# at-cg/PHI

Hardware: AMD Instinct MI355X
Metric: read Gbases/s scored (49-hap MHC graph stand-in synMHC-49); reads resident in HBM, parsing and H2D excluded (higher is better)
Workload: dtype u64

## Files before the change

phi_amd/csrc/contexts.hip:

```cpp
#include <hip/hip_runtime.h>
#include "phi_dev.h"
#include "phi_kernels.h"
#include "phi_wave.h"

static inline unsigned grid_for(int64_t n, int tpb)
{
    int64_t nb = (n + tpb - 1) / tpb;
    if (nb > 256 * 32) nb = 256 * 32;
    if (nb < 1) nb = 1;
    return (unsigned)nb;
}

#define GRID_STRIDE(i, n) \
    for (int64_t i = (int64_t)blockIdx.x * blockDim.x + threadIdx.x; i < (n); i += (int64_t)gridDim.x * blockDim.x)

__device__ __forceinline__ int32_t walk_of(const int64_t *__restrict__ walk_off, int32_t n_walks, int64_t e)
{
    int32_t lo = 0, hi = n_walks;
    while (hi - lo > 1) {
        const int32_t mid = (lo + hi) >> 1;
        if (walk_off[mid] <= e) lo = mid; else hi = mid;
    }
    return lo;
}

__global__ void __launch_bounds__(256) phi_vlen_kernel(const int64_t *__restrict__ seq_off, int64_t n_vtx, int32_t *__restrict__ vlen)
{
    GRID_STRIDE(v, n_vtx) vlen[v] = (int32_t)(seq_off[v + 1] - seq_off[v]);
}
void phi_launch_vlen(hipStream_t st, const int64_t *seq_off, int64_t n_vtx, int32_t *vlen)
{
    if (n_vtx > 0) hipLaunchKernelGGL(phi_vlen_kernel, dim3(grid_for(n_vtx, 256)), dim3(256), 0, st, seq_off, n_vtx, vlen);
}

template <bool BY_CLASS>
__global__ void __launch_bounds__(256) phi_walk_sum_kernel(const int32_t *__restrict__ key, const int32_t *__restrict__ val_of,
                                                           const int32_t *__restrict__ cls_rec_off, const int64_t *__restrict__ walk_off,
                                                           int32_t n_walks, int64_t n_entries, unsigned long long *__restrict__ out)
{
    const int64_t n_waves = (int64_t)gridDim.x * (blockDim.x / 64);
    const int64_t gw = (int64_t)blockIdx.x * (blockDim.x / 64) + (threadIdx.x >> 6);
    const int lane = threadIdx.x & 63;
    const int64_t per = ((n_entries + n_waves - 1) / n_waves + 63) & ~(int64_t)63;
    const int64_t lo = gw * per, hi = lo + per < n_entries ? lo + per : n_entries;
    if (lo >= hi) return;
    int32_t h = walk_of(walk_off, n_walks, lo);
    int64_t h_end = walk_off[h + 1];
    long long acc = 0;
    for (int64_t e0 = lo; e0 < hi; e0 += 64) {
        const int64_t e = e0 + lane;
        long long v = 0;
        if (e < hi) {
            const int32_t x = key[e];
            v = BY_CLASS ? (cls_rec_off[x + 1] - cls_rec_off[x]) : val_of[x];
        }
        if (e0 + 64 <= h_end) acc += v;
        else {
            int64_t row_lo = e0;
            for (;;) {
                const long long mine = (e >= row_lo && e < h_end) ? v : 0;
                acc += mine;
                if (h_end >= e0 + 64 || h_end >= hi) break;
                acc = phi_wave_sum(acc);
                if (lane == 0 && acc) atomicAdd(&out[h], (unsigned long long)acc);
                acc = 0;
                row_lo = h_end;
                h++;
                h_end = walk_off[h + 1];
            }
        }
    }
    acc = phi_wave_sum(acc);
    if (lane == 0 && acc) atomicAdd(&out[h], (unsigned long long)acc);
}
static inline unsigned walk_sum_grid(int64_t n_entries)
{
    int64_t nb = (n_entries + 256 * 64 - 1) / (256 * 64);
    if (nb > 1024) nb = 1024;
    return (unsigned)(nb < 1 ? 1 : nb);
}
void phi_launch_walk_bases(hipStream_t st, const int32_t *walk_vtx, const int32_t *vlen, const int64_t *walk_off, int32_t n_walks,
                           int64_t n_entries, unsigned long long *out)
{
    if (n_entries > 0)
        hipLaunchKernelGGL(phi_walk_sum_kernel<false>, dim3(walk_sum_grid(n_entries)), dim3(256), 0, st, walk_vtx, vlen, nullptr,
                           walk_off, n_walks, n_entries, out);
}
void phi_launch_walk_rec_counts(hipStream_t st, const int32_t *ent_cls, const int32_t *cls_rec_off, const int64_t *walk_off,
                                int32_t n_walks, int64_t n_entries, unsigned long long *out)
{
    if (n_entries > 0)
        hipLaunchKernelGGL(phi_walk_sum_kernel<true>, dim3(walk_sum_grid(n_entries)), dim3(256), 0, st, ent_cls, nullptr, cls_rec_off,
                           walk_off, n_walks, n_entries, out);
}

struct EntCtx { int32_t left; int32_t n; int32_t tail; };

__device__ __forceinline__ EntCtx entry_context(const PhiClassArgs &A, int64_t e, int64_t w_lo, int64_t w_hi)
{
    EntCtx c;
    c.left = 256;
    if (e > w_lo) {
        const int32_t pv = A.walk_vtx[e - 1];
        const int64_t pe = A.seq_off[pv + 1];
        c.left = pe > A.seq_off[pv] ? (int32_t)A.seq[pe - 1] : 257;
    }
    c.n = 0; c.tail = 0;
    while (c.tail < A.tail_need && e + c.n + 1 < w_hi) { c.n++; c.tail += A.vlen[A.walk_vtx[e + c.n]]; }
    return c;
}

__device__ __forceinline__ uint64_t context_key(const PhiClassArgs &A, int64_t e, const EntCtx &c)
{
    uint64_t h = A.seed ^ ((uint64_t)(uint32_t)c.left * 0x9E3779B97F4A7C15ull);
    h = phi_fmix64(h ^ (uint64_t)(uint32_t)c.n);
    for (int32_t j = 0; j <= c.n; j++) h = phi_fmix64(h ^ (uint64_t)(uint32_t)A.walk_vtx[e + j]) + 0x632BE59BD9B4E019ull;
    return h == PHI_EMPTY_KEY ? 0 : h;
}

__global__ void __launch_bounds__(256) phi_class_insert_kernel(PhiClassArgs A)
{
    GRID_STRIDE(e, A.n_entries) {
        const int32_t h = walk_of(A.walk_off, A.n_walks, e);
        const EntCtx c = entry_context(A, e, A.walk_off[h], A.walk_off[h + 1]);
        const uint64_t key = context_key(A, e, c);
        uint64_t s = key & A.t_mask;
        int probes = 0;
        for (;;) {
            unsigned long long prev = __builtin_nontemporal_load((const unsigned long long *)&A.t_keys[s]);
            if (prev == PHI_EMPTY_KEY) prev = atomicCAS((unsigned long long *)&A.t_keys[s], PHI_EMPTY_KEY, key);
            if (prev == PHI_EMPTY_KEY || prev == key) break;
            s = (s + 1) & A.t_mask;
            if (++probes > PHI_MAX_PROBE) { atomicOr(A.err, PHI_KERR_TABLE_FULL); break; }
        }
        if (__builtin_nontemporal_load(&A.t_rep[s]) > (uint32_t)e) atomicMin(&A.t_rep[s], (uint32_t)e);
        A.ent_slot[e] = (uint32_t)s;
    }
}

__global__ void __launch_bounds__(256) phi_class_verify_kernel(PhiClassArgs A, uint8_t *__restrict__ is_rep)
{
    GRID_STRIDE(e, A.n_entries) {
        const uint32_t s = A.ent_slot[e];
        const int64_t r = (int64_t)A.t_rep[s];
        is_rep[e] = r == e;
        if (r != e) {
            const int32_t h = walk_of(A.walk_off, A.n_walks, e), hr = walk_of(A.walk_off, A.n_walks, r);
            const int64_t w_hi = A.walk_off[h + 1], r_lo = A.walk_off[hr], r_hi = A.walk_off[hr + 1];
            const EntCtx c = entry_context(A, e, A.walk_off[h], w_hi);
            int32_t rleft = 256;
            if (r > r_lo) {
                const int32_t pv = A.walk_vtx[r - 1];
                const int64_t pe = A.seq_off[pv + 1];
                rleft = pe > A.seq_off[pv] ? (int32_t)A.seq[pe - 1] : 257;
            }
            bool same = rleft == c.left && r + c.n < r_hi;
            if (same && c.tail < A.tail_need && r + c.n + 1 != r_hi) same = false;
            for (int32_t j = 0; same && j <= c.n; j++) same = A.walk_vtx[r + j] == A.walk_vtx[e + j];
            if (!same) { atomicOr(A.err, PHI_KERR_FP_COLLISION); continue; }
        }
        atomicAdd(&A.t_mult[s], 1u);
    }
}

__global__ void __launch_bounds__(256) phi_class_ids_kernel(const phi_ent_t *__restrict__ cls_rep, int64_t n_cls,
                                                            const uint32_t *__restrict__ ent_slot, const uint32_t *__restrict__ t_mult,
                                                            uint32_t *__restrict__ t_cid, int32_t *__restrict__ cls_mult)
{
    GRID_STRIDE(c, n_cls) {
        const uint32_t s = ent_slot[cls_rep[c]];
        t_cid[s] = (uint32_t)c;
        cls_mult[c] = (int32_t)t_mult[s];
    }
}
__global__ void __launch_bounds__(256) phi_entry_class_kernel(const uint32_t *ent_slot, int64_t n_entries,
                                                              const uint32_t *__restrict__ t_cid, int32_t *ent_cls)
{
    GRID_STRIDE(e, n_entries) ent_cls[e] = (int32_t)t_cid[ent_slot[e]];
}

__global__ void __launch_bounds__(256) phi_class_len_kernel(PhiClassArgs A, const phi_ent_t *__restrict__ cls_rep, int64_t n_cls,
                                                            int32_t *__restrict__ cls_len, uint8_t *__restrict__ cls_left)
{
    GRID_STRIDE(c, n_cls) {
        const int64_t r = cls_rep[c];
        const int32_t h = walk_of(A.walk_off, A.n_walks, r);
        const EntCtx x = entry_context(A, r, A.walk_off[h], A.walk_off[h + 1]);
        const int32_t left = x.left != 256;
        cls_left[c] = (uint8_t)left;
        cls_len[c] = left + A.vlen[A.walk_vtx[r]] + (x.tail < A.tail_need ? x.tail : A.tail_need);
    }
}

void phi_launch_class_insert(hipStream_t st, const PhiClassArgs &A)
{
    if (A.n_entries > 0) hipLaunchKernelGGL(phi_class_insert_kernel, dim3(grid_for(A.n_entries, 256)), dim3(256), 0, st, A);
}
void phi_launch_class_verify(hipStream_t st, const PhiClassArgs &A, uint8_t *is_rep)
{
    if (A.n_entries > 0) hipLaunchKernelGGL(phi_class_verify_kernel, dim3(grid_for(A.n_entries, 256)), dim3(256), 0, st, A, is_rep);
}
void phi_launch_class_ids(hipStream_t st, const phi_ent_t *cls_rep, int64_t n_cls, const uint32_t *ent_slot, int64_t n_entries,
                          const uint32_t *t_mult, uint32_t *t_cid, int32_t *cls_mult, int32_t *ent_cls)
{
    if (n_cls > 0)
        hipLaunchKernelGGL(phi_class_ids_kernel, dim3(grid_for(n_cls, 256)), dim3(256), 0, st, cls_rep, n_cls, ent_slot, t_mult, t_cid, cls_mult);
    if (n_entries > 0)
        hipLaunchKernelGGL(phi_entry_class_kernel, dim3(grid_for(n_entries, 256)), dim3(256), 0, st, ent_slot, n_entries, t_cid, ent_cls);
}
void phi_launch_class_len(hipStream_t st, const PhiClassArgs &A, const phi_ent_t *cls_rep, int64_t n_cls, int32_t *cls_len, uint8_t *cls_left)
{
    if (n_cls > 0) hipLaunchKernelGGL(phi_class_len_kernel, dim3(grid_for(n_cls, 256)), dim3(256), 0, st, A, cls_rep, n_cls, cls_len, cls_left);
}

__global__ void __launch_bounds__(256) phi_pack_classes_kernel(const uint8_t *__restrict__ seq, const int64_t *__restrict__ seq_off,
                                                               const int32_t *__restrict__ walk_vtx, const int32_t *__restrict__ vlen,
                                                               const phi_ent_t *__restrict__ cls_rep, const uint8_t *__restrict__ cls_left,
                                                               const int64_t *__restrict__ cls_base, int64_t n_cls,
                                                               uint64_t *__restrict__ words, int64_t n_words, uint32_t *__restrict__ badbits,
                                                               uint8_t *__restrict__ ascii, unsigned long long *__restrict__ n_bad)
{
    const int64_t wi = (int64_t)blockIdx.x * blockDim.x + threadIdx.x;
    if (wi >= n_words + 4) return;
    if (wi >= n_words) {
        if (wi < n_words + 2) words[wi] = 0;
        if (badbits) badbits[wi] = 0;
        return;
    }
    const int64_t total = cls_base[n_cls];
    const int64_t b0 = wi * 32;
    uint64_t word = 0;
    uint32_t bad = 0;
    if (b0 < total) {
        int64_t c = phi_locate_in(cls_base, n_cls, b0);
        int64_t c_end = cls_base[c + 1];
        int64_t ent = -1, ent_o = 0, ent_end = 0;
        const uint8_t *src = nullptr;
        bool fresh = true;
        for (int j = 0; j < 32; j++) {
            const int64_t b = b0 + j;
            uint32_t ch = 'A';
            if (b < total) {
                while (b >= c_end) { c++; c_end = cls_base[c + 1]; fresh = true; }
                const int64_t o = b - cls_base[c];
                const int left = cls_left[c];
                if (left && o == 0) {
                    const int32_t pv = walk_vtx[cls_rep[c] - 1];
                    ch = seq[seq_off[pv + 1] - 1];
                } else {
                    if (fresh) {
                        ent = cls_rep[c]; ent_o = left;
                        const int32_t v = walk_vtx[ent];
                        ent_end = ent_o + vlen[v];
                        src = seq + seq_off[v] - ent_o;
                        fresh = false;
                    }
                    while (o >= ent_end) {
                        ent++; ent_o = ent_end;
                        const int32_t v = walk_vtx[ent];
                        ent_end = ent_o + vlen[v];
                        src = seq + seq_off[v] - ent_o;
                    }
                    ch = src[o];
                }
                bad |= (uint32_t)(!phi_is_acgt(ch)) << j;
                if (ascii) ascii[b] = (uint8_t)ch;
            }
            word = (word << 2) | phi_code(ch);
        }
    }
    words[wi] = word;
    if (badbits) badbits[wi] = bad;
    if (bad) atomicAdd(n_bad, (unsigned long long)__popc(bad));
}

void phi_launch_pack_classes(hipStream_t st, const uint8_t *seq, const int64_t *seq_off, const int32_t *walk_vtx, const int32_t *vlen,
                             const phi_ent_t *cls_rep, const uint8_t *cls_left, const int64_t *cls_base, int64_t n_cls, uint64_t *words,
                             int64_t n_words, uint32_t *badbits, uint8_t *ascii, unsigned long long *n_bad)
{
    if (n_words <= 0) return;
    const int64_t nb = (n_words + 4 + 255) / 256;
    hipLaunchKernelGGL(phi_pack_classes_kernel, dim3((unsigned)nb), dim3(256), 0, st, seq, seq_off, walk_vtx, vlen, cls_rep, cls_left,
                       cls_base, n_cls, words, n_words, badbits, ascii, n_bad);
// ... 313 lines not shown
```

phi_amd/csrc/phi_kernels.h:

```cpp
#pragma once
#include <stdint.h>
#include <hip/hip_runtime.h>
#include "phi_dp_flags.h"

#ifndef PHI_TPB
#define PHI_TPB 256

#endif
#define PHI_WCH 512
#define PHI_MAX_W 256
#define PHI_MAX_K 64
#define PHI_MAX_K_PACKED 32
#define PHI_MAX_PROBE 4096
#define PHI_RT_OVERFLOWED 1u
static inline int phi_nov_shift(int w)
{
    const int want = (3 * 2 * PHI_WCH) / (2 * (w + 1));
    int sh = 4;
    while ((1 << sh) < want && sh < 9) sh++;
    return sh;
}
#define PHI_STRIPES 256

typedef uint32_t phi_ent_t;
// ... 15 lines not shown
#define PHI_KERR_HASH_COLLISION 128u

struct PhiSketchArgs {
    const uint64_t *words;
    const unsigned long long *starts;
    int64_t n_bases;
    int32_t k, w;
    const unsigned long long *badbits;
    const uint8_t *ascii;
    int32_t allslow;
    int32_t *block_cnt;
    const int64_t *block_off;
    uint64_t *out_hash;
    int64_t *out_pos;
    unsigned long long *n_logged;
    unsigned long long *n_emitted;
    const uint64_t *u_rt; uint64_t u_bmask;
    uint8_t *hit;
    uint32_t *err;
    uint64_t *nov_log; uint16_t *nov_cnt; int64_t log_base; int32_t nov_shift;
    uint64_t *ov_list; unsigned long long *ov_count; int64_t ov_cap;
    const int64_t *read_off; int64_t n_reads;
    uint32_t reads_per_base_q32;
    int32_t uniform_len;
    double inv_len;
    uint32_t inv_len_q32;
    int32_t wave_stride;
    int32_t q_clean;
    int32_t win_reads;
    unsigned long long *ov_zero;
    unsigned long long *ipc_mb; unsigned long long ipc_scored, ipc_need;
    uint64_t *q_hit_words; int64_t q_n_hit_words; uint64_t *q_stripes; int64_t q_n_stripe_words;
    const uint64_t *k_rt; uint64_t k_bmask;
};
#define PHI_NOV_KMERS 0x8000u

void phi_launch_pack_ascii(hipStream_t st, const uint8_t *bases, int64_t n, uint64_t *words, int64_t n_words,
                           uint32_t *badbits, unsigned long long *n_bad);
void phi_launch_mark_starts(hipStream_t st, const int64_t *seq_off, int64_t n_seq, unsigned long long *starts);

void phi_launch_sketch_bytes(hipStream_t st, int mode, const PhiSketchArgs &A, const unsigned long long *batch_bad);
void phi_launch_reset_reads(hipStream_t st, uint64_t *hit_words, int64_t n_hit_words, uint64_t *stripes, int64_t n_stripe_words);
int64_t phi_sketch_num_blocks(int64_t n_bases);
int phi_sketch_win_reads(int k, int w, int64_t uniform_len, int64_t n_reads, int64_t n_bases);
int64_t phi_sketch_read_chunks(int k, int w, int64_t uniform_len, int64_t n_reads, int64_t n_bases);
void phi_launch_sketch(hipStream_t st, int mode, const PhiSketchArgs &A, hipEvent_t t0 = nullptr, hipEvent_t t1 = nullptr);

void phi_launch_table_build(hipStream_t st, const uint64_t *rec_hash, int64_t n_rec, uint64_t *u_keys,
                            uint32_t *u_rep, uint64_t u_mask, uint32_t *rec_slot, uint32_t *err);
void phi_launch_rep_flags(hipStream_t st, const uint32_t *rec_slot, int64_t n_rec, const uint32_t *u_rep,
                          uint8_t *flags);
void phi_launch_table_compact(hipStream_t st, const int32_t *rep_list, int64_t n_unique, const uint64_t *rec_hash, int64_t n_rec,
                              uint64_t *keys, uint32_t *uid, uint64_t mask, uint32_t *rec_slot, uint32_t *err);
void phi_launch_share_hist(hipStream_t st, const uint64_t *keys, int64_t cap, const int32_t *n_walks_of, unsigned long long *hist);
void phi_launch_slot_uid(hipStream_t st, const int32_t *rep_list, int64_t n_unique, const uint32_t *rec_slot,
                         uint32_t *u_uid);
void phi_launch_read_table(hipStream_t st, const uint64_t *keys, const uint32_t *uid, int64_t cap, uint64_t *rt,
                           int64_t n_buckets, uint32_t *err);
void phi_launch_fill_u64(hipStream_t st, uint64_t *p, int64_t n, uint64_t v);
void phi_launch_fill_u32(hipStream_t st, uint32_t *p, int64_t n, uint32_t v);
void phi_launch_iota_i64(hipStream_t st, int64_t *p, int64_t n, int64_t step);
void phi_launch_spectrum_insert(hipStream_t st, const uint64_t *hashes, int64_t n, uint64_t *sp_keys,
                                uint64_t sp_mask, unsigned long long *sp_count, const uint64_t *u_keys, uint64_t u_mask,
                                const uint32_t *u_uid, uint8_t *hit, uint32_t *err);
void phi_launch_spectrum_flush(hipStream_t st, const uint64_t *nov_log, const uint16_t *nov_cnt, int64_t c_lo, int64_t c_hi, int32_t shift,
                               uint64_t *sp_keys, uint64_t sp_mask, unsigned long long *sp_count, int32_t k, const uint64_t *u_keys,
                               uint64_t u_mask, uint32_t *err);
void phi_launch_kmer_keys(hipStream_t st, const int32_t *rec_cls, const int32_t *rec_rel, const uint64_t *rec_hash, const uint32_t *rec_slot,
                          int64_t n_rec, const int64_t *cls_base, const uint8_t *cls_left, const uint64_t *words, const uint32_t *badbits,
                          int32_t k, uint64_t *kkeys, unsigned long long *ctr);
void phi_launch_rt_overflowed(hipStream_t st, const uint64_t *rt, int64_t n_buckets, unsigned long long *n_out);
void phi_launch_count_flags(hipStream_t st, const uint8_t *flags, int64_t n, unsigned long long *n_out);
void phi_launch_spectrum_export(hipStream_t st, const uint64_t *sp_keys, int64_t cap, uint64_t *out,
                                unsigned long long *n_out);

struct PhiClassArgs {
    const int32_t *walk_vtx; const int64_t *walk_off; int32_t n_walks; int64_t n_entries;
    const int32_t *vlen; const uint8_t *seq; const int64_t *seq_off;
    int32_t tail_need;
    uint64_t seed;
    uint64_t *t_keys; uint32_t *t_rep; uint32_t *t_mult; uint64_t t_mask;
    uint32_t *ent_slot;
    uint32_t *err;
};
struct PhiExpandArgs {
    const int32_t *ent_cls; int64_t e_lo, e_hi;
    const int32_t *cls_rec_off; const phi_ent_t *cls_rep;
    const uint8_t *sel; const int32_t *sel_cnt;
    int32_t *block_cnt; const int64_t *block_off;
    const uint64_t *rec_hash; const int32_t *rec_rel; const int64_t *ent_base; uint64_t *out_hash; int64_t *out_pos;
    const uint32_t *rec_slot; const uint32_t *u_uid; const phi_ent_t *rec_e0; const phi_ent_t *rec_e1; uint32_t *out_tri;
};
void phi_launch_vlen(hipStream_t st, const int64_t *seq_off, int64_t n_vtx, int32_t *vlen);
void phi_launch_walk_bases(hipStream_t st, const int32_t *walk_vtx, const int32_t *vlen, const int64_t *walk_off, int32_t n_walks,
                           int64_t n_entries, unsigned long long *out);
void phi_launch_walk_rec_counts(hipStream_t st, const int32_t *ent_cls, const int32_t *cls_rec_off, const int64_t *walk_off,
                                int32_t n_walks, int64_t n_entries, unsigned long long *out);
void phi_launch_class_insert(hipStream_t st, const PhiClassArgs &A);
void phi_launch_class_verify(hipStream_t st, const PhiClassArgs &A, uint8_t *is_rep);
void phi_launch_class_ids(hipStream_t st, const phi_ent_t *cls_rep, int64_t n_cls, const uint32_t *ent_slot, int64_t n_entries,
                          const uint32_t *t_mult, uint32_t *t_cid, int32_t *cls_mult, int32_t *ent_cls);
void phi_launch_class_len(hipStream_t st, const PhiClassArgs &A, const phi_ent_t *cls_rep, int64_t n_cls, int32_t *cls_len, uint8_t *cls_left);
void phi_launch_pack_classes(hipStream_t st, const uint8_t *seq, const int64_t *seq_off, const int32_t *walk_vtx, const int32_t *vlen,
                             const phi_ent_t *cls_rep, const uint8_t *cls_left, const int64_t *cls_base, int64_t n_cls, uint64_t *words,
                             int64_t n_words, uint32_t *badbits, uint8_t *ascii, unsigned long long *n_bad);
void phi_launch_class_rec(hipStream_t st, const int64_t *raw_pos, int64_t n_raw, const int64_t *cls_base, int64_t n_cls,
                          const phi_ent_t *cls_rep, const uint8_t *cls_left, const int32_t *walk_vtx, const int32_t *vlen, int32_t k,
                          uint8_t *keep, int32_t *r_cls, int32_t *r_rel, phi_ent_t *r_e0, phi_ent_t *r_e1);
void phi_launch_class_rec_gather(hipStream_t st, const int32_t *idx, int64_t n, const uint64_t *raw_hash, const int32_t *r_cls,
                                 const int32_t *r_rel, const phi_ent_t *r_e0, const phi_ent_t *r_e1, uint64_t *o_hash, int32_t *o_cls,
                                 int32_t *o_rel, phi_ent_t *o_e0, phi_ent_t *o_e1);
void phi_launch_class_rec_off(hipStream_t st, const int32_t *rec_cls, int64_t n_rec, int64_t n_cls, int32_t *off);
int64_t phi_expand_num_blocks(int64_t n_entries);
void phi_launch_expand_count(hipStream_t st, const PhiExpandArgs &A);
void phi_launch_expand_write(hipStream_t st, const PhiExpandArgs &A, int kind);
void phi_launch_class_sel_count(hipStream_t st, const uint8_t *sel, const int32_t *cls_rec_off, int64_t n_cls, int32_t *sel_cnt);
void phi_launch_class_sel_tri(hipStream_t st, const uint8_t *sel, const int32_t *cls_rec_off, int64_t n_cls, const int32_t *sel_off, const phi_ent_t *cls_rep,
                              const uint32_t *rec_slot, const uint32_t *u_uid, const phi_ent_t *rec_e0, const phi_ent_t *rec_e1, int32_t *sel_tri);
void phi_launch_expand_tri(hipStream_t st, const int32_t *ent_cls, int64_t e_lo, int64_t e_hi, const int32_t *sel_off, const int32_t *sel_tri,
                           const int64_t *block_off, uint32_t *out_tri, phi_ent_t *a_e1, uint8_t *a_span, const int64_t *walk_off, int32_t n_walks,
                           unsigned long long *walk_cnt, unsigned long long *prep, int64_t n_anchors);
void phi_launch_mark_list(hipStream_t st, const int32_t *list, const int32_t *through, int64_t n, uint8_t *sel);
void phi_launch_share_count_cls(hipStream_t st, const int32_t *ent_cls, int64_t e_lo, int64_t e_hi, const int32_t *cls_rec_off,
                                const uint32_t *rec_slot, int32_t walk, int32_t *last_walk, int32_t *n_walks_of);
void phi_launch_entry_len_range(hipStream_t st, const int32_t *walk_vtx, const int32_t *vlen, int64_t e_lo, int64_t n, int32_t *lens);

#define PHI_KERR_FP_COLLISION 8u
void phi_launch_walk_edges(hipStream_t st, const int32_t *walk_vtx, const int64_t *walk_off, int32_t n_walks, int64_t n_entries, int32_t n_vtx,
                           const int64_t *adj_off, const int32_t *adj, const int64_t *seq_off, const int32_t *topo_rank,
                           uint8_t *e_out, int32_t *cnt_edge, unsigned long long *st_mask, int32_t nw64, int32_t *err);
void phi_launch_csr_count(hipStream_t st, const uint32_t *triples, int64_t n, int64_t n_ids, int32_t *cnt, uint32_t *err);
void phi_launch_csr_scatter(hipStream_t st, const uint32_t *triples, int64_t n, int64_t n_ids, const int32_t *off, int32_t *cur,
                            int32_t *idx);
void phi_launch_csr_sort(hipStream_t st, const int32_t *off, int64_t n_ids, int32_t *idx);
void phi_launch_match_flags(hipStream_t st, const uint32_t *rec_slot, int64_t n_rec, const uint32_t *u_uid,
                            const uint8_t *hit, uint8_t *flags);

struct PhiFilterArgs {
    const uint32_t *rec_slot; const phi_ent_t *rec_e0; const phi_ent_t *rec_e1;
    const int32_t *walk_vtx;
    const int32_t *rec_cls; const int32_t *cls_mult;
    const int32_t *m_rec;
    uint64_t *g_keys; int32_t *g_rep; uint32_t *g_cnt; uint64_t g_mask; uint64_t seed;
    int32_t *m_group;
    const uint32_t *u_uid;
    uint32_t *slot_maxcnt;
    uint8_t *slot_multi;
    float limit;
    unsigned long long *counters;
    uint32_t *err;
};
void phi_launch_group_insert(hipStream_t st, const PhiFilterArgs &A, int64_t n_matched);
void phi_launch_group_count(hipStream_t st, const PhiFilterArgs &A, int64_t n_matched);
void phi_launch_group_max(hipStream_t st, const PhiFilterArgs &A, int64_t n_matched);
void phi_launch_slot_count(hipStream_t st, const PhiFilterArgs &A, int64_t u_cap);
void phi_launch_kept_flags(hipStream_t st, const PhiFilterArgs &A, int64_t n_matched, uint8_t *kept, uint8_t *dp);
void phi_launch_gather_i32(hipStream_t st, const int32_t *src, const uint32_t *idx, int64_t n, int32_t *out);
void phi_launch_gather_u64(hipStream_t st, const uint64_t *src, const int32_t *idx, int64_t n, uint64_t *out);
void phi_launch_entry_csr(hipStream_t st, const phi_ent_t *a_e1, int64_t n_a, int64_t n_entries, int64_t *g_off);

#define PHI_DP_CHUNK 128
#define PHI_DP_RING 2048
#define PHI_SCOUT_MAX_WALKS 65535
#define PHI_DP_MAX_WALKS 1022

struct PhiDpArgs {
    int32_t n_vtx, n_walks;
    const int32_t *st_rec;
    const unsigned long long *st_mask;
    const int32_t *in_packed;
    const int64_t *walk_off;
    const uint64_t *word;
    const int64_t *g_off; const uint8_t *g_span; const uint8_t *a_weight;
    int32_t cost;
    int32_t *dmax;
    int32_t *bstart;
    int32_t *tops;
    int32_t *ent_src, *ent_h;
};
void phi_launch_dp(hipStream_t st, const PhiDpArgs &A);
int phi_dp_num_waves(int n_walks);
void phi_launch_dp_words(hipStream_t st, const uint8_t *e_out, const int64_t *g_off, const uint8_t *g_span,
// ... 131 lines not shown
```

phi_amd/csrc/set_graph.hip:

```cpp
#include <string.h>
#include <algorithm>
#include <future>
#include <memory>
#include "phi_ctx.h"
#include "phi_dev.h"
#include "dp_steps.h"

static int build_read_table(phi_ctx *c)
{
    uint64_t nb = pow2_at_least(std::max<uint64_t>(64, (16 * (uint64_t)c->n_unique + 2) / 3));
    if (const char *e = getenv("PHI_READ_TABLE_BUCKETS")) nb = pow2_at_least(std::max<long long>(atoll(e), 1));
    uint32_t err0 = 0;
    HIPCHK(hipMemcpyAsync(&err0, scalar(c, S_ERR), 4, hipMemcpyDeviceToHost, c->stream));
    HIPCHK(hipStreamSynchronize(c->stream));
    for (int attempt = 0;; attempt++) {
        PHICHK(phi_dev_ensure(c, c->d_rt, nb * 32));
        phi_launch_read_table(c->stream, c->d_u_keys.as<uint64_t>(), c->d_u_uid.as<uint32_t>(), (int64_t)c->u_cap,
                              c->d_rt.as<uint64_t>(), (int64_t)nb, (uint32_t *)scalar(c, S_ERR));
        uint32_t err = 0;
        HIPCHK(hipMemcpyAsync(&err, scalar(c, S_ERR), 4, hipMemcpyDeviceToHost, c->stream));
        HIPCHK(hipStreamSynchronize(c->stream));
        if ((err0 & PHI_KERR_TABLE_FULL) || !(err & PHI_KERR_TABLE_FULL)) break;
        if (attempt >= 40) return phi_fail(c, PHI_ERR_OVERFLOW, "read table overflow at %llu buckets (internal error)", (unsigned long long)nb);
        err &= ~PHI_KERR_TABLE_FULL;
        HIPCHK(phi_copy_sync(c, scalar(c, S_ERR), &err, 4, hipMemcpyHostToDevice));
        nb *= 2;
    }
    c->rt_buckets = nb; c->rt_mask = nb - 1;
    return PHI_OK;
}

static int build_kmer_table(phi_ctx *c)
{
    c->kt_buckets = 0; c->kt_mask = 0;
    if (c->k > 31 || c->n_rec <= 0 || c->n_unique <= 0) return PHI_OK;
    PhiStageTimer tg("set_graph");
    DevBuf kkeys, ctr;
    PhiDevGuard guard{{&kkeys, &ctr}};
    PHICHK(phi_dev_ensure(c, kkeys, c->u_cap * 8));
    PHICHK(phi_dev_ensure(c, ctr, 5 * 8));
    phi_launch_fill_u64(c->stream, kkeys.as<uint64_t>(), (int64_t)c->u_cap, PHI_EMPTY_KEY);
    HIPCHK(hipMemsetAsync(ctr.p, 0, 5 * 8, c->stream));
    phi_launch_kmer_keys(c->stream, c->d_rec_cls.as<int32_t>(), c->d_rec_rel.as<int32_t>(), c->d_rec_hash.as<uint64_t>(), c->d_rec_slot.as<uint32_t>(),
                         c->n_rec, c->d_cls_base.as<int64_t>(), c->d_cls_left.as<uint8_t>(), c->d_wwords.as<uint64_t>(), c->d_wbad.as<uint32_t>(),
                         c->k, kkeys.as<uint64_t>(), ctr.as<unsigned long long>());
    uint64_t n[5] = {0, 0, 0, 0, 0};
    HIPCHK(phi_copy_sync(c, n, ctr.p, 3 * 8, hipMemcpyDeviceToHost));
    if (n[1]) return phi_fail(c, PHI_ERR_DEVICE, "k-mer table: %llu class records whose k-mer in class space does not hash to the record's hash (internal error)", (unsigned long long)n[1]);
    if (n[2]) {
        if (tg.on) fprintf(stderr, "[phi timing] set_graph: %llu walk minimisers share a hash with another k-mer: no k-mer table for this graph\n", (unsigned long long)n[2]);
        return PHI_OK;
    }
    uint64_t nb = c->rt_buckets;
    uint32_t err0 = 0;
    HIPCHK(phi_copy_sync(c, &err0, scalar(c, S_ERR), 4, hipMemcpyDeviceToHost));
    if (err0 & PHI_KERR_TABLE_FULL) return PHI_OK;
    for (int attempt = 0;; attempt++) {
        PHICHK(phi_dev_ensure(c, c->d_kt, nb * 32));
        phi_launch_read_table(c->stream, kkeys.as<uint64_t>(), c->d_u_uid.as<uint32_t>(), (int64_t)c->u_cap, c->d_kt.as<uint64_t>(), (int64_t)nb,
                              (uint32_t *)scalar(c, S_ERR));
        uint32_t err = 0;
        HIPCHK(phi_copy_sync(c, &err, scalar(c, S_ERR), 4, hipMemcpyDeviceToHost));
        if (!(err & PHI_KERR_TABLE_FULL)) break;
        if (attempt >= 40) return phi_fail(c, PHI_ERR_OVERFLOW, "k-mer table overflow at %llu buckets (internal error)", (unsigned long long)nb);
        err &= ~PHI_KERR_TABLE_FULL;
        HIPCHK(phi_copy_sync(c, scalar(c, S_ERR), &err, 4, hipMemcpyHostToDevice));
        nb *= 2;
    }
    c->kt_buckets = nb; c->kt_mask = nb - 1;
    int n_cu = 0;
    HIPCHK(hipDeviceGetAttribute(&n_cu, hipDeviceAttributeMultiprocessorCount, c->device));
    c->kt_max_chunks = (int64_t)n_cu * 4 * 7;
    if (tg.on) {
        phi_launch_rt_overflowed(c->stream, c->d_rt.as<uint64_t>(), (int64_t)c->rt_buckets, ctr.as<unsigned long long>() + 3);
        phi_launch_rt_overflowed(c->stream, c->d_kt.as<uint64_t>(), (int64_t)nb, ctr.as<unsigned long long>() + 4);
        HIPCHK(phi_copy_sync(c, n + 3, ctr.as<uint64_t>() + 3, 2 * 8, hipMemcpyDeviceToHost));
        fprintf(stderr, "[phi timing] set_graph: k-mer table of %llu buckets (%.1f MB) beside the read table's %llu; %llu class records with a base outside ACGT skipped; "
                        "OVERFLOWED buckets: read table %.2e, k-mer table %.2e\n", (unsigned long long)nb, (double)nb * 32 / 1e6, (unsigned long long)c->rt_buckets,
                (unsigned long long)n[0], (double)n[3] / (double)c->rt_buckets, (double)n[4] / (double)nb);
        tg.lap("[gpu thread]   k-mer table");
    }
    return PHI_OK;
}

static int build_classes(phi_ctx *c, int32_t n_vtx, int32_t n_walks, int64_t n_entries)
{
    PhiStageTimer tg("set_graph");
    hipEvent_t ev0 = nullptr, ev1 = nullptr;
    HIPCHK(hipEventCreate(&ev0));
    HIPCHK(hipEventCreate(&ev1));
    struct EvGuard { hipEvent_t a, b; ~EvGuard() { (void)hipEventDestroy(a); (void)hipEventDestroy(b); } } evg{ev0, ev1};
    HIPCHK(hipEventRecord(ev0, c->stream));
    PHICHK(phi_dev_ensure(c, c->d_vlen, (size_t)n_vtx * 4));
    phi_launch_vlen(c->stream, c->d_seq_off.as<int64_t>(), n_vtx, c->d_vlen.as<int32_t>());
    PHICHK(phi_dev_ensure(c, c->d_list, (size_t)(n_walks + 1) * 8));
    HIPCHK(hipMemsetAsync(c->d_list.p, 0, (size_t)(n_walks + 1) * 8, c->stream));
    phi_launch_walk_bases(c->stream, c->d_walk_vtx.as<int32_t>(), c->d_vlen.as<int32_t>(), c->d_walk_off.as<int64_t>(), n_walks, n_entries,
                          c->d_list.as<unsigned long long>());
    c->h_walk_base.assign(n_walks + 1, 0);
    HIPCHK(hipMemcpyAsync(c->h_walk_base.data() + 1, c->d_list.p, (size_t)n_walks * 8, hipMemcpyDeviceToHost, c->stream));

    tg.lap("[gpu thread]     events, vlen, walk bases");
    PHICHK(phi_dev_ensure(c, c->d_ent_cls, (size_t)n_entries * 4));
    PHICHK(phi_dev_ensure(c, c->d_flags, (size_t)n_entries));
    DevBuf t_keys, t_rep, t_mult;
    PhiDevGuard guard{{&t_keys, &t_rep, &t_mult}};
    PhiClassArgs A{};
    A.walk_vtx = c->d_walk_vtx.as<int32_t>(); A.walk_off = c->d_walk_off.as<int64_t>(); A.n_walks = n_walks; A.n_entries = n_entries;
    A.vlen = c->d_vlen.as<int32_t>(); A.seq = c->d_seq.as<uint8_t>(); A.seq_off = c->d_seq_off.as<int64_t>();
    A.tail_need = c->w + c->k - 2;
    A.ent_slot = c->d_ent_cls.as<uint32_t>();
    A.err = (uint32_t *)scalar(c, S_ERR);
    const uint64_t cap_max = pow2_at_least(std::max<uint64_t>(1024, 2 * (uint64_t)n_entries));
    uint64_t cap = std::min(cap_max, pow2_at_least(std::max<uint64_t>(1024, 4 * (uint64_t)n_vtx)));
    tg.lap("[gpu thread]     entry buffers");
    for (int attempt = 0;; attempt++) {
        PHICHK(phi_dev_ensure(c, t_keys, cap * 8));
        PHICHK(phi_dev_ensure(c, t_rep, cap * 4));
        PHICHK(phi_dev_ensure(c, t_mult, cap * 4));
        A.t_keys = t_keys.as<uint64_t>(); A.t_rep = t_rep.as<uint32_t>(); A.t_mult = t_mult.as<uint32_t>(); A.t_mask = cap - 1;
        A.seed = 0x13198A2E03707344ull + 0x9E3779B97F4A7C15ull * (uint64_t)attempt;
        phi_launch_fill_u64(c->stream, A.t_keys, (int64_t)cap, PHI_EMPTY_KEY);
        phi_launch_fill_u32(c->stream, A.t_rep, (int64_t)cap, 0xFFFFFFFFu);
        HIPCHK(hipMemsetAsync(A.t_mult, 0, cap * 4, c->stream));
        phi_launch_class_insert(c->stream, A);
        uint32_t err = 0;
        HIPCHK(hipMemcpyAsync(&err, scalar(c, S_ERR), 4, hipMemcpyDeviceToHost, c->stream));
        HIPCHK(hipStreamSynchronize(c->stream));
        if (err & PHI_KERR_TABLE_FULL) {
            if (cap == cap_max) return phi_fail(c, PHI_ERR_OVERFLOW, "walk-context table overflow (internal error)");
            cap = std::min(cap_max, cap * 8);
            err &= ~PHI_KERR_TABLE_FULL;
            HIPCHK(phi_copy_sync(c, scalar(c, S_ERR), &err, 4, hipMemcpyHostToDevice));
            attempt--;
            continue;
        }
        phi_launch_class_verify(c->stream, A, c->d_flags.as<uint8_t>());
        HIPCHK(hipMemcpyAsync(&err, scalar(c, S_ERR), 4, hipMemcpyDeviceToHost, c->stream));
        HIPCHK(hipStreamSynchronize(c->stream));
        if (!(err & PHI_KERR_FP_COLLISION)) break;
        if (attempt >= 7) return phi_fail(c, PHI_ERR_DEVICE, "walk-context fingerprints collide under 8 seeds (internal error)");
        err &= ~PHI_KERR_FP_COLLISION;
        HIPCHK(phi_copy_sync(c, scalar(c, S_ERR), &err, 4, hipMemcpyHostToDevice));
    }
    tg.lap("[gpu thread]     table insert + verify");
    for (int32_t h = 0; h < n_walks; h++) c->h_walk_base[h + 1] += c->h_walk_base[h];
    c->walk_bases = c->h_walk_base[n_walks];
    PHICHK(phi_compact(c, c->d_flags.as<uint8_t>(), n_entries, c->d_cls_rep, &c->n_cls));
    const int64_t nc = c->n_cls;
    tg.lap("[gpu thread]     compact representatives");
    PHICHK(phi_dev_ensure(c, c->d_cls_mult, (size_t)nc * 4));
    PHICHK(phi_dev_ensure(c, c->d_cls_left, (size_t)nc));
    PHICHK(phi_dev_ensure(c, c->d_cls_base, (size_t)(nc + 1) * 8));
    PHICHK(phi_dev_ensure(c, c->d_cls_rec_off, (size_t)(nc + 1) * 4));
    phi_launch_class_ids(c->stream, c->d_cls_rep.as<phi_ent_t>(), nc, A.ent_slot, n_entries, A.t_mult, A.t_rep, c->d_cls_mult.as<int32_t>(),
                         c->d_ent_cls.as<int32_t>());
    PHICHK(phi_dev_ensure(c, c->d_list3, (size_t)nc * 4));
    phi_launch_class_len(c->stream, A, c->d_cls_rep.as<phi_ent_t>(), nc, c->d_list3.as<int32_t>(), c->d_cls_left.as<uint8_t>());
    PHICHK(phi_scan(c, c->d_list3.as<int32_t>(), nc, c->d_cls_base.as<int64_t>()));
    int64_t run = 0;
    HIPCHK(hipMemcpyAsync(&run, c->d_cls_base.as<int64_t>() + nc, 8, hipMemcpyDeviceToHost, c->stream));
    HIPCHK(hipStreamSynchronize(c->stream));
    c->cls_bases = run;
    if (tg.on) fprintf(stderr, "[phi timing] set_graph: %lld entries in %lld classes, %lld bases of class space for %lld bases of walks\\n",
                       (long long)n_entries, (long long)nc, (long long)run, (long long)c->walk_bases);
    tg.lap("[gpu thread]   classes");

    const int64_t n_words = (run + 31) / 32;
    PHICHK(phi_dev_ensure(c, c->d_wwords, (size_t)(n_words + 2) * 8));
    PHICHK(phi_dev_ensure(c, c->d_wbad, (size_t)(n_words + 6) * 4));
    auto pack = [&](uint8_t *ascii) {
        phi_launch_pack_classes(c->stream, c->d_seq.as<uint8_t>(), c->d_seq_off.as<int64_t>(), c->d_walk_vtx.as<int32_t>(), c->d_vlen.as<int32_t>(),
                                c->d_cls_rep.as<phi_ent_t>(), c->d_cls_left.as<uint8_t>(), c->d_cls_base.as<int64_t>(), nc,
                                c->d_wwords.as<uint64_t>(), n_words, c->d_wbad.as<uint32_t>(), ascii, (unsigned long long *)scalar(c, S_NBAD));
    };
    pack(nullptr);
    const uint8_t *cls_ascii = nullptr;
    {
        uint64_t n_bad = 0;
        HIPCHK(hipMemcpyAsync(&n_bad, scalar(c, S_NBAD), 8, hipMemcpyDeviceToHost, c->stream));
        HIPCHK(hipStreamSynchronize(c->stream));
        if (n_bad || c->k > PHI_MAX_K_PACKED) {
            PHICHK(phi_dev_ensure(c, c->d_wascii, (size_t)run + 64));
            HIPCHK(hipMemsetAsync(scalar(c, S_NBAD), 0, 8, c->stream));
            pack(c->d_wascii.as<uint8_t>());
            cls_ascii = c->d_wascii.as<uint8_t>();
        }
    }
    const size_t n_sw = (size_t)(run / 64 + 2);
    PHICHK(phi_dev_ensure(c, c->d_wstarts, n_sw * 8));
    HIPCHK(hipMemsetAsync(c->d_wstarts.p, 0, n_sw * 8, c->stream));
    phi_launch_mark_starts(c->stream, c->d_cls_base.as<int64_t>(), nc, c->d_wstarts.as<unsigned long long>());
    int64_t n_raw = 0;
    DevBuf raw_hash;
    PhiDevGuard guard1{{&raw_hash}};
    PHICHK(sketch_records(c, c->d_wwords.as<uint64_t>(), c->d_wstarts.as<unsigned long long>(), run, c->k, c->w, cls_ascii, raw_hash,
                          c->d_rec_pos, &n_raw));
    if (n_raw >= (int64_t)1 << 31) return phi_fail(c, PHI_ERR_UNSUPPORTED, "more than 2^31 minimisers in the distinct walk contexts");
    tg.lap("[gpu thread]   class-space pack + sketch");

    const int64_t nr0 = std::max<int64_t>(n_raw, 1);
    DevBuf r_cls, r_rel, r_e0, r_e1;
    PhiDevGuard guard4{{&r_cls, &r_rel, &r_e0, &r_e1}};
    PHICHK(phi_dev_ensure(c, r_cls, (size_t)nr0 * 4));
    PHICHK(phi_dev_ensure(c, r_rel, (size_t)nr0 * 4));
    PHICHK(phi_dev_ensure(c, r_e0, (size_t)nr0 * 4));
    PHICHK(phi_dev_ensure(c, r_e1, (size_t)nr0 * 4));
    PHICHK(phi_dev_ensure(c, c->d_flags, (size_t)std::max<int64_t>(nr0, n_entries)));
    phi_launch_class_rec(c->stream, c->d_rec_pos.as<int64_t>(), n_raw, c->d_cls_base.as<int64_t>(), nc, c->d_cls_rep.as<phi_ent_t>(),
                         c->d_cls_left.as<uint8_t>(), c->d_walk_vtx.as<int32_t>(), c->d_vlen.as<int32_t>(), c->k, c->d_flags.as<uint8_t>(),
                         r_cls.as<int32_t>(), r_rel.as<int32_t>(), r_e0.as<phi_ent_t>(), r_e1.as<phi_ent_t>());
    PHICHK(phi_compact(c, c->d_flags.as<uint8_t>(), n_raw, c->d_list2, &c->n_rec));
    const int64_t nr = std::max<int64_t>(c->n_rec, 1);
    PHICHK(phi_dev_ensure(c, c->d_rec_hash, (size_t)nr * 8));
    PHICHK(phi_dev_ensure(c, c->d_rec_cls, (size_t)nr * 4));
    PHICHK(phi_dev_ensure(c, c->d_rec_rel, (size_t)nr * 4));
    PHICHK(phi_dev_ensure(c, c->d_rec_e0, (size_t)nr * 4));
    PHICHK(phi_dev_ensure(c, c->d_rec_e1, (size_t)nr * 4));
    phi_launch_class_rec_gather(c->stream, c->d_list2.as<int32_t>(), c->n_rec, raw_hash.as<uint64_t>(), r_cls.as<int32_t>(), r_rel.as<int32_t>(),
                                r_e0.as<phi_ent_t>(), r_e1.as<phi_ent_t>(), c->d_rec_hash.as<uint64_t>(), c->d_rec_cls.as<int32_t>(),
                                c->d_rec_rel.as<int32_t>(), c->d_rec_e0.as<phi_ent_t>(), c->d_rec_e1.as<phi_ent_t>());
    phi_launch_class_rec_off(c->stream, c->d_rec_cls.as<int32_t>(), c->n_rec, nc, c->d_cls_rec_off.as<int32_t>());
    HIPCHK(hipEventRecord(ev1, c->stream));
    HIPCHK(hipStreamSynchronize(c->stream));
    float ms = 0.f;
    HIPCHK(hipEventElapsedTime(&ms, ev0, ev1));
    c->index_gpu_ms = ms;
    HIPCHK(hipGetLastError());
    return PHI_OK;
}

int set_graph_check_args(phi_ctx *c, int32_t n_vtx, const char *seq_concat, const int64_t *seq_off, const int64_t *adj_off,
                         const int32_t *adj, int32_t n_walks, const int64_t *walk_off, const int32_t *walk_vtx, const int32_t *topo_rank)
{
    const bool dev_walks = walk_vtx == nullptr;
    if (dev_walks && c && walk_off && n_walks > 0 && !(c->walks_on_device && c->walks_on_device_n == walk_off[n_walks] && (int32_t)(c->wtext.ends.size() / 2) == n_walks))
        return phi_fail(c, PHI_ERR_STATE, "phi_set_graph without walk_vtx: phi_walk_text_resolve must have resolved exactly these walks on this context");
    if (n_vtx <= 0 || n_walks <= 0 || !seq_concat || !seq_off || !adj_off || !walk_off || !topo_rank)
        return phi_fail(c, PHI_ERR_INVALID, "phi_set_graph: null pointer or empty graph");
    if (adj_off[n_vtx] > 0 && !adj) return phi_fail(c, PHI_ERR_INVALID, "phi_set_graph: adj is null");
    HIPCHK(hipSetDevice(c->device));
    if (c->ipc) return phi_fail(c, PHI_ERR_STATE, "phi_set_graph on a context in a group of processes: phi_ipc_destroy first (the peers have this context's hit vectors mapped)");
    c->have_graph = false;
    c->chop.on = false;
    c->panel.on = false;
    phi_scout_end(c);
    c->solved = false;
    phi_ladder_drop(c);
// ... 464 lines not shown
```

Before: 479.8.

## Compute walk-context class keys per tile with shared-memory prefix hashes

Replaces the per-entry walk-context class insert with a tiled kernel. Each block stages vertex lengths and position-weighted hash terms for a tile plus halo in shared memory. Block scans over those terms then give each entry's context length and an invertible multiplicative rolling hash, which replaces the per-entry walks and per-vertex sequence lookups. A packed vinfo array (length plus last base) is added, and verification becomes a tiled kernel launched right after insert, removing one host sync round-trip. This is set_graph preprocessing, so it probably does not touch the timed read-scoring throughput.

```diff
diff --git a/phi_amd/csrc/contexts.hip b/phi_amd/csrc/contexts.hip
--- a/phi_amd/csrc/contexts.hip
+++ b/phi_amd/csrc/contexts.hip
@@ -24,13 +24,18 @@
     return lo;
 }
 
-__global__ void __launch_bounds__(256) phi_vlen_kernel(const int64_t *__restrict__ seq_off, int64_t n_vtx, int32_t *__restrict__ vlen)
-{
-    GRID_STRIDE(v, n_vtx) vlen[v] = (int32_t)(seq_off[v + 1] - seq_off[v]);
-}
-void phi_launch_vlen(hipStream_t st, const int64_t *seq_off, int64_t n_vtx, int32_t *vlen)
-{
-    if (n_vtx > 0) hipLaunchKernelGGL(phi_vlen_kernel, dim3(grid_for(n_vtx, 256)), dim3(256), 0, st, seq_off, n_vtx, vlen);
+__global__ void __launch_bounds__(256) phi_vlen_kernel(const int64_t *__restrict__ seq_off, const uint8_t *__restrict__ seq, int64_t n_vtx,
+                                                       int32_t *__restrict__ vlen, uint32_t *__restrict__ vinfo)
+{
+    GRID_STRIDE(v, n_vtx) {
+        const int64_t lo = seq_off[v], hi = seq_off[v + 1];
+        vlen[v] = (int32_t)(hi - lo);
+        if (vinfo) vinfo[v] = (uint32_t)(hi - lo < 0xFFFFFF ? hi - lo : 0xFFFFFF) | (hi > lo ? (uint32_t)seq[hi - 1] << 24 : 0u);
+    }
+}
+void phi_launch_vlen(hipStream_t st, const int64_t *seq_off, const uint8_t *seq, int64_t n_vtx, int32_t *vlen, uint32_t *vinfo)
+{
+    if (n_vtx > 0) hipLaunchKernelGGL(phi_vlen_kernel, dim3(grid_for(n_vtx, 256)), dim3(256), 0, st, seq_off, seq, n_vtx, vlen, vinfo);
 }
 
 template <bool BY_CLASS>
@@ -163,6 +168,140 @@
     }
 }
 
+constexpr uint64_t ct_pow(uint64_t b, unsigned e) { uint64_t r = 1; for (; e; e >>= 1, b *= b) if (e & 1) r *= b; return r; }
+constexpr uint64_t ct_inverse(uint64_t a) { uint64_t x = a; for (int i = 0; i < 6; i++) x *= 2 - a * x; return x; }
+constexpr uint64_t CT_M = 0x9E3779B97F4A7C15ull, CT_MINV = ct_inverse(CT_M);
+static_assert(CT_M * CT_MINV == 1, "M^-1 mod 2^64");
+#define CT_STAGED (PHI_CLASS_TILE_MAX + PHI_CLASS_HALO_MAX + 2)
+#define CT_DESC_N(d) ((int)((d) >> 9) & 511)
+
+__device__ __forceinline__ uint64_t ct_pow_dev(uint64_t b, unsigned e)
+{
+    uint64_t r = 1;
+    for (; e; e >>= 1, b *= b) if (e & 1) r *= b;
+    return r;
+}
+
+__global__ void __launch_bounds__(256) phi_class_tile_insert_kernel(PhiClassArgs A)
+{
+    __shared__ int32_t s_len[CT_STAGED];
+    __shared__ uint64_t s_pre[CT_STAGED];
+    __shared__ uint16_t s_left[PHI_CLASS_TILE_MAX];
+    __shared__ int32_t s_wl[4];
+    __shared__ uint64_t s_wp[4];
+    __shared__ int64_t s_walk[3];
+    const int t = threadIdx.x, T = A.tile, H = A.tail_need, S = T + H + 1;
+    const int C = (S + 1 + 255) / 256;
+    const uint64_t pw_t = ct_pow_dev(CT_M, (unsigned)t), inv_t = ct_pow_dev(CT_MINV, (unsigned)t + 1);
+    const int64_t n_tiles = (A.n_entries + T - 1) / T;
+    for (int64_t tile = blockIdx.x; tile < n_tiles; tile += gridDim.x) {
+        const int64_t e0 = tile * T;
+        if (t == 0) {
+            const int32_t h = walk_of(A.walk_off, A.n_walks, e0);
+            s_walk[0] = h; s_walk[1] = A.walk_off[h]; s_walk[2] = A.walk_off[h + 1];
+        }
+        uint64_t pw = pw_t;
+        for (int i = t; i <= S; i += 256, pw *= ct_pow(CT_M, 256)) {
+            const int64_t g = e0 - 1 + i;
+            int32_t len = 0;
+            uint32_t left = 257;
+            uint64_t term = 0;
+            if (i < S && g >= 0 && g < A.n_entries) {
+                const int32_t v = A.walk_vtx[g];
+                const uint32_t info = A.vinfo[v];
+                const int32_t l = (int32_t)(info & 0xFFFFFF);
+                len = l < H ? l : H;
+                if (l) left = info >> 24;
+                term = phi_fmix64(A.seed ^ (uint64_t)(uint32_t)v) * pw;
+            }
+            s_len[i] = len; s_pre[i] = term;
+            if (i < T) s_left[i] = (uint16_t)left;
+        }
+        __syncthreads();
+        {
+            const int lo = t * C, hi = lo + C < S + 1 ? lo + C : S + 1;
+            int32_t sl = 0;
+            uint64_t sp = 0;
+            for (int i = lo; i < hi; i++) { sl += s_len[i]; sp += s_pre[i]; }
+            int32_t rl = phi_block_excl_scan<4>(sl, s_wl);
+            uint64_t rp = phi_block_excl_scan<4>(sp, s_wp);
+            for (int i = lo; i < hi; i++) {
+                const int32_t l = s_len[i];
+                const uint64_t p = s_pre[i];
+                s_len[i] = rl; s_pre[i] = rp;
+                rl += l; rp += p;
+            }
+        }
+        __syncthreads();
+        const int32_t h0 = (int32_t)s_walk[0];
+        uint64_t inv = inv_t;
+        for (int a = t; a < T; a += 256, inv *= ct_pow(CT_MINV, 256)) {
+            const int64_t e = e0 + a;
+            if (e >= A.n_entries) break;
+            int64_t w_lo = s_walk[1], w_hi = s_walk[2];
+            if (e >= w_hi) {
+                int32_t lo = h0, hi = A.n_walks;
+                while (hi - lo > 1) {
+                    const int32_t mid = (lo + hi) >> 1;
+                    if (A.walk_off[mid] <= e) lo = mid; else hi = mid;
+                }
+                w_lo = A.walk_off[lo]; w_hi = A.walk_off[lo + 1];
+            }
+            const int i = a + 1;
+            const uint32_t left = e > w_lo ? s_left[a] : 256u;
+            const int n_max = w_hi - e - 1 < H ? (int)(w_hi - e - 1) : H;
+            const int32_t base = s_len[i + 1];
+            int n = 0, tail = 0;
+            while (tail < H && n < n_max) { n++; tail = s_len[i + 1 + n] - base; }
+            const uint32_t desc = left | (uint32_t)n << 9 | (uint32_t)(tail < H) << 18;
+            const uint64_t comb = (s_pre[i + n + 1] - s_pre[i]) * inv;
+            uint64_t key = phi_fmix64(comb ^ ((uint64_t)desc * 0xD6E8FEB86659FD93ull)) & A.key_mask;
+            if (key == PHI_EMPTY_KEY) key = 0;
+            uint64_t s = key & A.t_mask;
+            int probes = 0;
+            for (;;) {
+                unsigned long long prev = __builtin_nontemporal_load((const unsigned long long *)&A.t_keys[s]);
+                if (prev == PHI_EMPTY_KEY) prev = atomicCAS((unsigned long long *)&A.t_keys[s], PHI_EMPTY_KEY, key);
+                if (prev == PHI_EMPTY_KEY || prev == key) break;
+                s = (s + 1) & A.t_mask;
+                if (++probes > PHI_MAX_PROBE) { atomicOr(A.err, PHI_KERR_TABLE_FULL); break; }
+            }
+            if (__builtin_nontemporal_load(&A.t_rep[s]) > (uint32_t)e) atomicMin(&A.t_rep[s], (uint32_t)e);
+            if (A.count_in_insert) atomicAdd(&A.t_mult[s], 1u);
+            A.ent_slot[e] = (uint32_t)s;
+            A.ent_desc[e] = desc;
+        }
+        __syncthreads();
+    }
+}
+
+__global__ void __launch_bounds__(256) phi_class_tile_verify_kernel(PhiClassArgs A, uint8_t *__restrict__ is_rep)
+{
+    __shared__ int32_t s_vtx[PHI_CLASS_TILE_MAX + PHI_CLASS_HALO_MAX];
+    const int t = threadIdx.x, T = A.tile, H = A.tail_need, S = T + H;
+    const int64_t n_tiles = (A.n_entries + T - 1) / T;
+    for (int64_t tile = blockIdx.x; tile < n_tiles; tile += gridDim.x) {
+        const int64_t e0 = tile * T;
+        for (int i = t; i < S; i += 256) s_vtx[i] = e0 + i < A.n_entries ? A.walk_vtx[e0 + i] : -1;
+        __syncthreads();
+        for (int a = t; a < T; a += 256) {
+            const int64_t e = e0 + a;
+            if (e >= A.n_entries) break;
+            const uint32_t s = A.ent_slot[e];
+            const int64_t r = (int64_t)A.t_rep[s];
+            is_rep[e] = r == e;
+            if (r != e) {
+                const uint32_t d = A.ent_desc[e];
+                bool same = r < A.n_entries && A.ent_desc[r] == d;
+                for (int j = 0, n = CT_DESC_N(d); same && j <= n; j++) same = A.walk_vtx[r + j] == s_vtx[a + j];
+                if (!same) { atomicOr(A.err, PHI_KERR_FP_COLLISION); continue; }
+            }
+            if (!A.count_in_insert) atomicAdd(&A.t_mult[s], 1u);
+        }
+        __syncthreads();
+    }
+}
+
 __global__ void __launch_bounds__(256) phi_class_ids_kernel(const phi_ent_t *__restrict__ cls_rep, int64_t n_cls,
                                                             const uint32_t *__restrict__ ent_slot, const uint32_t *__restrict__ t_mult,
                                                             uint32_t *__restrict__ t_cid, int32_t *__restrict__ cls_mult)
@@ -199,6 +338,14 @@
 void phi_launch_class_verify(hipStream_t st, const PhiClassArgs &A, uint8_t *is_rep)
 {
     if (A.n_entries > 0) hipLaunchKernelGGL(phi_class_verify_kernel, dim3(grid_for(A.n_entries, 256)), dim3(256), 0, st, A, is_rep);
+}
+void phi_launch_class_tiles(hipStream_t st, const PhiClassArgs &A, uint8_t *is_rep)
+{
+    if (A.n_entries <= 0) return;
+    int64_t nb = (A.n_entries + A.tile - 1) / A.tile;
+    if (nb > 256 * 8) nb = 256 * 8;
+    hipLaunchKernelGGL(phi_class_tile_insert_kernel, dim3((unsigned)nb), dim3(256), 0, st, A);
+    hipLaunchKernelGGL(phi_class_tile_verify_kernel, dim3((unsigned)nb), dim3(256), 0, st, A, is_rep);
 }
 void phi_launch_class_ids(hipStream_t st, const phi_ent_t *cls_rep, int64_t n_cls, const uint32_t *ent_slot, int64_t n_entries,
                           const uint32_t *t_mult, uint32_t *t_cid, int32_t *cls_mult, int32_t *ent_cls)
diff --git a/phi_amd/csrc/phi_kernels.h b/phi_amd/csrc/phi_kernels.h
--- a/phi_amd/csrc/phi_kernels.h
+++ b/phi_amd/csrc/phi_kernels.h
@@ -121,7 +121,14 @@
     uint64_t *t_keys; uint32_t *t_rep; uint32_t *t_mult; uint64_t t_mask;
     uint32_t *ent_slot;
     uint32_t *err;
-};
+    const uint32_t *vinfo;
+    uint32_t *ent_desc;
+    int32_t tile;
+    uint64_t key_mask;
+    int32_t count_in_insert;
+};
+#define PHI_CLASS_TILE_MAX 1024
+#define PHI_CLASS_HALO_MAX (PHI_MAX_W + PHI_MAX_K - 2)
 struct PhiExpandArgs {
     const int32_t *ent_cls; int64_t e_lo, e_hi;
     const int32_t *cls_rec_off; const phi_ent_t *cls_rep;
@@ -130,13 +137,14 @@
     const uint64_t *rec_hash; const int32_t *rec_rel; const int64_t *ent_base; uint64_t *out_hash; int64_t *out_pos;
     const uint32_t *rec_slot; const uint32_t *u_uid; const phi_ent_t *rec_e0; const phi_ent_t *rec_e1; uint32_t *out_tri;
 };
-void phi_launch_vlen(hipStream_t st, const int64_t *seq_off, int64_t n_vtx, int32_t *vlen);
+void phi_launch_vlen(hipStream_t st, const int64_t *seq_off, const uint8_t *seq, int64_t n_vtx, int32_t *vlen, uint32_t *vinfo);
 void phi_launch_walk_bases(hipStream_t st, const int32_t *walk_vtx, const int32_t *vlen, const int64_t *walk_off, int32_t n_walks,
                            int64_t n_entries, unsigned long long *out);
 void phi_launch_walk_rec_counts(hipStream_t st, const int32_t *ent_cls, const int32_t *cls_rec_off, const int64_t *walk_off,
                                 int32_t n_walks, int64_t n_entries, unsigned long long *out);
 void phi_launch_class_insert(hipStream_t st, const PhiClassArgs &A);
 void phi_launch_class_verify(hipStream_t st, const PhiClassArgs &A, uint8_t *is_rep);
+void phi_launch_class_tiles(hipStream_t st, const PhiClassArgs &A, uint8_t *is_rep);
 void phi_launch_class_ids(hipStream_t st, const phi_ent_t *cls_rep, int64_t n_cls, const uint32_t *ent_slot, int64_t n_entries,
                           const uint32_t *t_mult, uint32_t *t_cid, int32_t *cls_mult, int32_t *ent_cls);
 void phi_launch_class_len(hipStream_t st, const PhiClassArgs &A, const phi_ent_t *cls_rep, int64_t n_cls, int32_t *cls_len, uint8_t *cls_left);
diff --git a/phi_amd/csrc/set_graph.hip b/phi_amd/csrc/set_graph.hip
--- a/phi_amd/csrc/set_graph.hip
+++ b/phi_amd/csrc/set_graph.hip
@@ -91,8 +91,16 @@
     HIPCHK(hipEventCreate(&ev1));
     struct EvGuard { hipEvent_t a, b; ~EvGuard() { (void)hipEventDestroy(a); (void)hipEventDestroy(b); } } evg{ev0, ev1};
     HIPCHK(hipEventRecord(ev0, c->stream));
+    const bool per_entry = getenv("PHI_CLASS_PER_ENTRY") != nullptr;
+    int tile = PHI_CLASS_TILE_MAX, fp_bits = 64;
+    if (const char *e = getenv("PHI_CLASS_TILE")) tile = std::min(std::max(atoi(e), 1), PHI_CLASS_TILE_MAX);
+    if (const char *e = getenv("PHI_CLASS_FP_BITS")) fp_bits = std::min(std::max(atoi(e), 1), 64);
+    const char *count_env = getenv("PHI_CLASS_COUNT");
+    DevBuf t_keys, t_rep, t_mult, vinfo, ent_desc;
+    PhiDevGuard guard{{&t_keys, &t_rep, &t_mult, &vinfo, &ent_desc}};
     PHICHK(phi_dev_ensure(c, c->d_vlen, (size_t)n_vtx * 4));
-    phi_launch_vlen(c->stream, c->d_seq_off.as<int64_t>(), n_vtx, c->d_vlen.as<int32_t>());
+    if (!per_entry) PHICHK(phi_dev_ensure(c, vinfo, (size_t)n_vtx * 4));
+    phi_launch_vlen(c->stream, c->d_seq_off.as<int64_t>(), c->d_seq.as<uint8_t>(), n_vtx, c->d_vlen.as<int32_t>(), vinfo.as<uint32_t>());
     PHICHK(phi_dev_ensure(c, c->d_list, (size_t)(n_walks + 1) * 8));
     HIPCHK(hipMemsetAsync(c->d_list.p, 0, (size_t)(n_walks + 1) * 8, c->stream));
     phi_launch_walk_bases(c->stream, c->d_walk_vtx.as<int32_t>(), c->d_vlen.as<int32_t>(), c->d_walk_off.as<int64_t>(), n_walks, n_entries,
@@ -103,18 +111,21 @@
     tg.lap("[gpu thread]     events, vlen, walk bases");
     PHICHK(phi_dev_ensure(c, c->d_ent_cls, (size_t)n_entries * 4));
     PHICHK(phi_dev_ensure(c, c->d_flags, (size_t)n_entries));
-    DevBuf t_keys, t_rep, t_mult;
-    PhiDevGuard guard{{&t_keys, &t_rep, &t_mult}};
+    if (!per_entry) PHICHK(phi_dev_ensure(c, ent_desc, (size_t)n_entries * 4));
     PhiClassArgs A{};
     A.walk_vtx = c->d_walk_vtx.as<int32_t>(); A.walk_off = c->d_walk_off.as<int64_t>(); A.n_walks = n_walks; A.n_entries = n_entries;
     A.vlen = c->d_vlen.as<int32_t>(); A.seq = c->d_seq.as<uint8_t>(); A.seq_off = c->d_seq_off.as<int64_t>();
     A.tail_need = c->w + c->k - 2;
     A.ent_slot = c->d_ent_cls.as<uint32_t>();
     A.err = (uint32_t *)scalar(c, S_ERR);
+    A.vinfo = vinfo.as<uint32_t>(); A.ent_desc = ent_desc.as<uint32_t>(); A.tile = tile;
+    A.count_in_insert = !(count_env && !strcmp(count_env, "verify"));
     const uint64_t cap_max = pow2_at_least(std::max<uint64_t>(1024, 2 * (uint64_t)n_entries));
     uint64_t cap = std::min(cap_max, pow2_at_least(std::max<uint64_t>(1024, 4 * (uint64_t)n_vtx)));
     tg.lap("[gpu thread]     entry buffers");
+    int n_attempts = 0;
     for (int attempt = 0;; attempt++) {
+        n_attempts++;
         PHICHK(phi_dev_ensure(c, t_keys, cap * 8));
         PHICHK(phi_dev_ensure(c, t_rep, cap * 4));
         PHICHK(phi_dev_ensure(c, t_mult, cap * 4));
@@ -123,21 +134,25 @@
         phi_launch_fill_u64(c->stream, A.t_keys, (int64_t)cap, PHI_EMPTY_KEY);
         phi_launch_fill_u32(c->stream, A.t_rep, (int64_t)cap, 0xFFFFFFFFu);
         HIPCHK(hipMemsetAsync(A.t_mult, 0, cap * 4, c->stream));
-        phi_launch_class_insert(c->stream, A);
+        A.key_mask = attempt == 0 && fp_bits < 64 ? ((uint64_t)1 << fp_bits) - 1 : ~(uint64_t)0;
         uint32_t err = 0;
+        if (per_entry) phi_launch_class_insert(c->stream, A);
+        else phi_launch_class_tiles(c->stream, A, c->d_flags.as<uint8_t>());
         HIPCHK(hipMemcpyAsync(&err, scalar(c, S_ERR), 4, hipMemcpyDeviceToHost, c->stream));
         HIPCHK(hipStreamSynchronize(c->stream));
         if (err & PHI_KERR_TABLE_FULL) {
             if (cap == cap_max) return phi_fail(c, PHI_ERR_OVERFLOW, "walk-context table overflow (internal error)");
             cap = std::min(cap_max, cap * 8);
-            err &= ~PHI_KERR_TABLE_FULL;
+            err &= ~(PHI_KERR_TABLE_FULL | PHI_KERR_FP_COLLISION);
             HIPCHK(phi_copy_sync(c, scalar(c, S_ERR), &err, 4, hipMemcpyHostToDevice));
             attempt--;
             continue;
         }
-        phi_launch_class_verify(c->stream, A, c->d_flags.as<uint8_t>());
-        HIPCHK(hipMemcpyAsync(&err, scalar(c, S_ERR), 4, hipMemcpyDeviceToHost, c->stream));
-        HIPCHK(hipStreamSynchronize(c->stream));
+        if (per_entry) {
+            phi_launch_class_verify(c->stream, A, c->d_flags.as<uint8_t>());
+            HIPCHK(hipMemcpyAsync(&err, scalar(c, S_ERR), 4, hipMemcpyDeviceToHost, c->stream));
+            HIPCHK(hipStreamSynchronize(c->stream));
+        }
         if (!(err & PHI_KERR_FP_COLLISION)) break;
         if (attempt >= 7) return phi_fail(c, PHI_ERR_DEVICE, "walk-context fingerprints collide under 8 seeds (internal error)");
         err &= ~PHI_KERR_FP_COLLISION;
@@ -162,8 +177,10 @@
     HIPCHK(hipMemcpyAsync(&run, c->d_cls_base.as<int64_t>() + nc, 8, hipMemcpyDeviceToHost, c->stream));
     HIPCHK(hipStreamSynchronize(c->stream));
     c->cls_bases = run;
-    if (tg.on) fprintf(stderr, "[phi timing] set_graph: %lld entries in %lld classes, %lld bases of class space for %lld bases of walks\\n",
-                       (long long)n_entries, (long long)nc, (long long)run, (long long)c->walk_bases);
+    if (tg.on) fprintf(stderr, "[phi timing] set_graph: %lld entries in %lld classes, %lld bases of class space for %lld bases of walks; "
+                               "class table: %d attempt%s, %llu slots (%s)\n",
+                       (long long)n_entries, (long long)nc, (long long)run, (long long)c->walk_bases, n_attempts, n_attempts == 1 ? "" : "s",
+                       (unsigned long long)cap, per_entry ? "entry by entry" : "tiles");
     tg.lap("[gpu thread]   classes");
 
     const int64_t n_words = (run + 31) / 32;
```

New measurement: 475.5. No clear change (-0.9%).
